# aquaskyline/SOAPdenovo-Trans

Hardware: AMD Instinct MI355X
Metric: pregraph k-mers hashed/sec (higher is better)
Workload: dtype u64

## Files before the change

### soapdenovo-trans_amd/csrc/sdt_pipeline.hip

```cpp
#include "sdt_ctx.hpp"
#include "sdt_tile.cuh"
#include "sdt_superkmer_kernels.cuh"
#include "sdt_count_plan.h"
#include "sdt_pipeline.hpp"

void sk_free(sdt_ctx *c)
{
	sdt_ctx::SkState &k = c->sk;
	void *dev[] = {k.p1.recs, k.p1.meta, k.p1.next, k.p2.recs, k.p2.meta, k.p2.next, k.cursors, k.blk, k.cnt1, k.off1, k.fill1, k.list1,
	               k.cnt2, k.off2, k.fill2, k.list2, k.kmers2, k.kpre2, k.items, k.citems, k.next_item};
	for (void *p : dev)
		if (p) (void)hipFree(p);
	void *host[] = {k.h_off1, k.h_off2, k.h_kpre2, k.h_items, k.h_citems};
	for (void *p : host)
		if (p) (void)hipHostFree(p);
	const uint64_t in_total = k.l2_in_total;
	const bool exchanged = k.exchanged;
	const uint32_t stream_flushes = k.stream_flushes;
	k = sdt_ctx::SkState();
	k.l2_in_total = in_total;
	k.exchanged = exchanged;
	k.stream_flushes = stream_flushes;
}

// ... 29 lines not shown

int sk_reset_pool1(sdt_ctx *c)
{
	sdt_ctx::SkState &k = c->sk;
	HIPCHK(hipMemsetAsync(k.p1.next, 0, 4, c->stream));
	HIPCHK(hipMemsetAsync(k.cnt1, 0, SK_NB1 * 4, c->stream));
	hipLaunchKernelGGL(k_sk_init_cursors, dim3(256), dim3(256), 0, c->stream, k.cursors, k.wgs * (uint32_t)SK_NB1, (uint32_t)SK_CAP1, k.blk, k.wgs);
	HIPCHK(hipGetLastError());
	k.pending_kmers = 0;
	return SDT_OK;
}

int sk_alloc(sdt_ctx *c, uint64_t want_kmers, uint64_t per_read)
{
	sdt_ctx::SkState &k = c->sk;
	if (want_kmers > SK_BATCH_MAX_KMERS)
		want_kmers = SK_BATCH_MAX_KMERS;
	if (k.ready && (k.cap_kmers >= want_kmers || k.cap_is_max || k.pending_kmers))
		return SDT_OK;
	if (k.ready) {
		HIPCHK(hipStreamSynchronize(c->stream));
		sk_free(c);
	}
	const int rw = sk_rec_words(c->nw), rw2 = sk_rec2_stride(c->nw);
	const int w = c->K - sk_minimizer_len(c->K) + 1;
	const double rate = 2.0 / (double)(w + 1) + 1.0 / (double)sk_max_run(c->K, c->nw);
	double run = 1.0 / rate * ((c->nw == 4 || per_read > (uint64_t)SK_SEQ_MAX_KMERS) ? 0.8 : 1.0);
	if (run > (double)per_read) run = (double)per_read;
	uint64_t div = (uint64_t)run;
	if (div < 2) div = 2;
	div = (uint64_t)clamp_int(sdt_knob_int(sdt_tuning_env("SDT_SK_POOL_DIV"), (int)div), 1, 1 << 20);
	const int mem_pct = sdt_knob_int(sdt_tuning_env("SDT_SK_POOL_MEM_PCT"), 70);
	size_t free_b = 0, total_b = 0;
	HIPCHK(sdti::mem_info(&free_b, &total_b));
	uint64_t cap = want_kmers < (1ULL << 24) ? (1ULL << 24) : want_kmers;
	k.cap_is_max = cap >= SK_BATCH_MAX_KMERS;
	const uint32_t wgs = (uint32_t)c->cu_count * 6;
	for (;; cap /= 2) {
		const uint64_t recs = cap / div;
		const uint64_t chunks1 = sdt_knob_int(sdt_test_env("SDT_SK_POOL_CHUNKS1"), 0) > 0 ? (uint64_t)sdt_knob_int(sdt_test_env("SDT_SK_POOL_CHUNKS1"), 0) : recs / SK_CAP1 + (uint64_t)wgs * SK_NB1 + 1024;
		const uint64_t items = chunks1 / SK_ITEM_CHUNKS + SK_NB1 + 1;
		const uint64_t chunks2 = chunks1 * (SK_CAP1 / SK_CAP2) + items * (SK_NB2 + SK_BLK2) + 1024;
		const uint64_t bytes = chunks1 * SK_CAP1 * rw * 8 + chunks2 * SK_CAP2 * rw2 * 8 + (chunks1 + chunks2) * 8;
		const uint64_t all = c->comm.nranks > 1 ? bytes + chunks1 * SK_CAP1 * rw * 8 * 9 / 2 : bytes;
		if (chunks2 >= (1ULL << SK_LIST2_FILL_SHIFT) - 1 || all > free_b / 100 * (uint64_t)mem_pct) {
			k.cap_is_max = true;
			if (cap <= (1ULL << 24))
				return fail(SDT_ENOMEM, "super-k-mer pools: %llu MiB needed for the smallest batch, %zu MiB free",
				            (unsigned long long)(bytes >> 20), free_b >> 20);
			continue;
		}
		k.p1.chunks = (uint32_t)chunks1;
		k.p2.chunks = (uint32_t)chunks2;
		k.items_cap = (uint32_t)items;
		break;
	}
	k.wgs = wgs;
	const double t_alloc0 = comm_now();
	HIPCHK(hipMalloc((void **)&k.p1.recs, (size_t)k.p1.chunks * SK_CAP1 * rw * 8));
	HIPCHK(hipMalloc((void **)&k.p1.meta, (size_t)k.p1.chunks * 4));
	HIPCHK(hipMalloc((void **)&k.p1.next, 64));
	HIPCHK(hipMalloc((void **)&k.p2.recs, (size_t)k.p2.chunks * SK_CAP2 * rw2 * 8));
// ... 8 lines not shown
	HIPCHK(hipMalloc((void **)&k.cnt2, SK_NBF * 4));
	HIPCHK(hipMalloc((void **)&k.off2, (SK_NBF + 1) * 4));
	HIPCHK(hipMalloc((void **)&k.fill2, SK_NBF * 4));
	HIPCHK(hipMalloc((void **)&k.list2, (size_t)k.p2.chunks * 4));
	HIPCHK(hipMalloc((void **)&k.kmers2, SK_NBF * 8));
	HIPCHK(hipMalloc((void **)&k.kpre2, (SK_NBF + 1) * 8));
	HIPCHK(hipMalloc((void **)&k.items, (size_t)k.items_cap * sizeof(SkItem)));
	HIPCHK(hipHostMalloc((void **)&k.h_off1, (SK_NB1 + 1) * 4, hipHostMallocDefault));
	HIPCHK(hipHostMalloc((void **)&k.h_off2, (SK_NBF + 1) * 4, hipHostMallocDefault));
	HIPCHK(hipHostMalloc((void **)&k.h_kpre2, (SK_NBF + 1) * 8, hipHostMallocDefault));
	HIPCHK(hipHostMalloc((void **)&k.h_items, (size_t)k.items_cap * sizeof(SkItem), hipHostMallocDefault));
	k.citems_cap = (uint32_t)SK_NBF + k.p2.chunks / SK_COUNT_ITEM_CHUNKS + 1;
	HIPCHK(hipMalloc((void **)&k.citems, (size_t)k.citems_cap * sizeof(uint4)));
	HIPCHK(hipHostMalloc((void **)&k.h_citems, (size_t)k.citems_cap * sizeof(uint4), hipHostMallocDefault));
	HIPCHK(hipMalloc((void **)&k.next_item, SK_MAX_COUNT_LAUNCHES * sizeof(uint32_t)));
	k.cap_kmers = cap;
	k.ready = true;
	if (sdt_env("SDT_TIMING"))
		fprintf(stderr, "[libsdt_gpu] super-k-mer pools for %llu k-mers per batch: %.1f GiB in %.0f ms\n", (unsigned long long)cap,
		        ((double)k.p1.chunks * SK_CAP1 * rw + (double)k.p2.chunks * SK_CAP2 * rw2) * 8 / (1 << 30), (comm_now() - t_alloc0) * 1e3);
	return sk_reset_pool1(c);
}

template <int NW, bool TRACK> static int sk_launch_count_t(sdt_ctx *c, uint32_t i0, uint32_t i1, uint32_t launch)
{
	sdt_ctx::SkState &k = c->sk;
	const size_t smem = sk_count_smem<NW, TRACK>();
	const unsigned per_cu = (unsigned)((160 * 1024) / (smem + 256));
	unsigned grid = (unsigned)c->cu_count * (per_cu < 1 ? 1 : (per_cu > 2 ? 2 : per_cu));
	if (grid > i1 - i0) grid = i1 - i0;
	HIPCHK(hipFuncSetAttribute((const void *)k_sk_count<NW, TRACK>, hipFuncAttributeMaxDynamicSharedMemorySize, (int)smem));
	hipLaunchKernelGGL((k_sk_count<NW, TRACK>), dim3(grid), dim3(SkCntGeo<NW, TRACK>::TPB), smem, c->stream, k.p2, k.list2, (const uint4 *)k.citems, i0, i1,
	                   k.next_item + launch, c->K, flat_of<NW>(c), c->d_stats);
	HIPCHK(hipGetLastError());
	return SDT_OK;
}

template <int NW> static int sk_launch_count(sdt_ctx *c, uint32_t i0, uint32_t i1, uint32_t launch)
{
	return c->d_first ? sk_launch_count_t<NW, true>(c, i0, i1, launch) : sk_launch_count_t<NW, false>(c, i0, i1, launch);
}


int sk_list1(sdt_ctx *c)
{
	sdt_ctx::SkState &k = c->sk;
	const int g = c->cu_count * 8;
	hipLaunchKernelGGL(k_sk_seal, dim3(256), dim3(256), 0, c->stream, k.cursors, k.wgs * (uint32_t)SK_NB1, k.blk, k.wgs, k.p1, (uint32_t)SK_CAP1);
	hipLaunchKernelGGL(k_sk_scan, dim3(1), dim3(1024), 0, c->stream, k.cnt1, k.off1, k.fill1, (int)SK_NB1, (const unsigned long long *)nullptr, (unsigned long long *)nullptr);
	hipLaunchKernelGGL(k_sk_chunk_place_few, dim3(g), dim3(256), 0, c->stream, k.p1, k.off1, k.fill1, k.list1, (int)SK_NB1);
	SK_CHK(hipGetLastError());
	SK_CHK(hipMemcpyAsync(k.h_off1, k.off1, (SK_NB1 + 1) * 4, hipMemcpyDeviceToHost, c->stream));
	{ const int rcw = c->comm.sync_watched(c->stream, "the chunk lists of a round"); if (rcw != SDT_OK) return rcw; }
	k.st_chunks1 = k.h_off1[SK_NB1];
	return SDT_OK;
}

int sk_split(sdt_ctx *c, const SkPool &src, const uint32_t *list, uint32_t nitems, hipEvent_t after_l2)
{
	sdt_ctx::SkState &k = c->sk;
	const int g = c->cu_count * 8;
	SK_CHK(hipMemsetAsync(k.p2.next, 0, 4, c->stream));
	SK_CHK(hipMemsetAsync(k.kmers2, 0, SK_NBF * 8, c->stream));
	SK_CHK(hipMemsetAsync(k.cnt2, 0, SK_NBF * 4, c->stream));
	if (nitems) {
		SK_CHK(hipMemcpyAsync(k.items, k.h_items, (size_t)nitems * sizeof(SkItem), hipMemcpyHostToDevice, c->stream));
		const size_t sm = c->nw == 1 ? SkL2Stage<1>::SMEM : (c->nw == 2 ? SkL2Stage<2>::SMEM : SkL2Stage<4>::SMEM);
		const void *fn = c->nw == 1 ? (const void *)k_sk_scatter_records_staged<1> : (c->nw == 2 ? (const void *)k_sk_scatter_records_staged<2> : (const void *)k_sk_scatter_records_staged<4>);
		SK_CHK(hipFuncSetAttribute(fn, hipFuncAttributeMaxDynamicSharedMemorySize, (int)sm));
		if (c->nw == 1) hipLaunchKernelGGL(k_sk_scatter_records_staged<1>, dim3(nitems), dim3(SK_L2S_TPB), sm, c->stream, src, list, k.items, k.p2, k.cnt2, k.kmers2, c->d_stats);
		else if (c->nw == 2) hipLaunchKernelGGL(k_sk_scatter_records_staged<2>, dim3(nitems), dim3(SK_L2S_TPB), sm, c->stream, src, list, k.items, k.p2, k.cnt2, k.kmers2, c->d_stats);
		else hipLaunchKernelGGL(k_sk_scatter_records_staged<4>, dim3(nitems), dim3(SK_L2S_TPB), sm, c->stream, src, list, k.items, k.p2, k.cnt2, k.kmers2, c->d_stats);
		SK_CHK(hipGetLastError());
	}
	if (after_l2)
		SK_CHK(hipEventRecord(after_l2, c->stream));
	hipLaunchKernelGGL(k_sk_scan, dim3(1), dim3(1024), 0, c->stream, k.cnt2, k.off2, k.fill2, (int)SK_NBF, (const unsigned long long *)k.kmers2, k.kpre2);
	hipLaunchKernelGGL(k_sk_chunk_place, dim3(g), dim3(256), 0, c->stream, k.p2, k.off2, k.fill2, k.list2);
	SK_CHK(hipGetLastError());
	SK_CHK(hipMemcpyAsync(k.h_kpre2, k.kpre2, (SK_NBF + 1) * 8, hipMemcpyDeviceToHost, c->stream));
	SK_CHK(hipMemcpyAsync(k.h_off2, k.off2, (SK_NBF + 1) * 4, hipMemcpyDeviceToHost, c->stream));
	return SDT_OK;
}

int sk_count_all(sdt_ctx *c)
{
	sdt_ctx::SkState &k = c->sk;
	SK_CHK(hipStreamSynchronize(c->stream));
	k.st_chunks2 = k.h_off2[SK_NBF];
	k.st_flushes++;
	k.stream_flushes++;
	k.l2_in_total += k.h_kpre2[SK_NBF];
	int rc = SDT_OK;
	uint32_t nci = 0;
	SK_CHK(hipMemsetAsync(k.next_item, 0, SK_MAX_COUNT_LAUNCHES * sizeof(uint32_t), c->stream));
// ... 101 lines not shown
		k.pending_kmers = 0;
		rc = sk_count_all(c);
	}
	if (hipEventRecord(ev2->b, c->stream) != hipSuccess && rc == SDT_OK)
		rc = fail(SDT_EHIP, "hipEventRecord failed");
	k.flushing = false;
	return rc;
}

template <int NW> static Table<NW> sk_tbl(const sdt_ctx *c, bool allow_direct)
{
	Table<NW> t = flat_of<NW>(c);
	if (!allow_direct)
		t.ent = nullptr;
	return t;
}

int sk_scatter_launch(sdt_ctx *c, const uint32_t *d_words, const uint64_t *d_offs, uint64_t nr, uint64_t max_read_len, uint64_t ob,
                             bool allow_direct)
{
	sdt_ctx::SkState &k = c->sk;
	const uint64_t per_read = max_read_len - c->K + 1;
	const SkGeo geo = sk_geo(c->K, max_read_len);
	const int m = sk_minimizer_len(c->K), ncap = sk_max_run(c->K, c->nw);
	const uint64_t ntiles = (nr + SK_TILE_READS - 1) / SK_TILE_READS;
	const unsigned grid = (unsigned)(ntiles < k.wgs ? ntiles : k.wgs);
	EventPair *ev = next_event(c);
	if (!ev)
		return fail(SDT_EHIP, "hipEventCreate failed");
	ev->kmers = nr * per_read;
	ev->stage = SDT_STAGE_SK_SCATTER;
	HIPCHK(hipEventRecord(ev->a, c->stream));
#define SK_SCATTER(NW)                                                                                                             \
	do {                                                                                                                       \
		HIPCHK(hipFuncSetAttribute((const void *)k_sk_scatter_reads<NW>, hipFuncAttributeMaxDynamicSharedMemorySize, (int)geo.smem)); \
		hipLaunchKernelGGL(k_sk_scatter_reads<NW>, dim3(grid), dim3(TPB), geo.smem, c->stream, d_words, d_offs, nr, c->K, m, ncap, \
		                   geo.mtw, geo.tile_words, geo.hv_words, geo.hv2_words, geo.bits_words, k.p1, k.cursors, k.blk, k.cnt1, sk_tbl<NW>(c, allow_direct), c->d_stats, ob, c->ord_stride); \
	} while (0)
	const int w = c->K - m + 1;
	static const bool no_seq = sdt_tuning_env("SDT_SK_STRIPS") != NULL;
	const bool seq1 = c->nw == 1 && (w & 1) && w >= 9 && w <= 21 && per_read <= (uint64_t)SK_SEQ_MAX_KMERS;
	const bool seq2 = c->nw == 2 && (w & 1) && w >= 23 && w <= 53 && per_read <= (uint64_t)SK_SEQ_MAX_KMERS;
	if ((seq1 || seq2) && !no_seq) {
		SkSeqLaunch a;
		a.words = d_words; a.offs = d_offs; a.nreads = nr; a.K = c->K; a.m = m; a.ncap = ncap;
		a.mtw = (int)(((uint64_t)SK_SEQ_TILE * max_read_len + 16 + 15) / 16) + TAIL_PAD + 1;
		a.pool = k.p1; a.cursors = k.cursors; a.blk = k.blk; a.cnt = k.cnt1; a.stats = c->d_stats;
		a.ord_base = ob; a.ord_stride = c->ord_stride; a.max_wgs = k.wgs; a.cu_count = c->cu_count; a.stream = c->stream;
		HIPCHK(seq1 ? sk_seq_launch_nw1(w, a, sk_tbl<1>(c, allow_direct)) : (w <= 33 ? sk_seq_launch_nw2_lo(w, a, sk_tbl<2>(c, allow_direct))
		            : (w <= 43 ? sk_seq_launch_nw2_mid(w, a, sk_tbl<2>(c, allow_direct)) : sk_seq_launch_nw2_hi(w, a, sk_tbl<2>(c, allow_direct)))));
	} else if (c->nw == 1) SK_SCATTER(1);
	else if (c->nw == 2) SK_SCATTER(2);
	else SK_SCATTER(4);
#undef SK_SCATTER
	HIPCHK(hipGetLastError());
	HIPCHK(hipEventRecord(ev->b, c->stream));
	k.pending_kmers += nr * per_read;
	return SDT_OK;
}
// ... 105 lines not shown
```

### soapdenovo-trans_amd/csrc/sdt_pipeline.hpp

```cpp
#pragma once
#include "sdt_ctx.hpp"

static const uint64_t SK_BATCH_MAX_KMERS = 1ULL << clamp_int(sdt_knob_int(sdt_size_env("SDT_SK_BATCH_LOG2"), 35), 24, 36);
static const uint32_t SK_ITEM_CHUNKS = (uint32_t)clamp_int(sdt_knob_int(sdt_size_env("SDT_SK_ITEM_CHUNKS"), 4096), 16, 4096);
static const uint64_t SK_COUNT_KMERS = 1ULL << clamp_int(sdt_knob_int(sdt_size_env("SDT_SK_COUNT_KMERS_LOG2"), 29), 20, 36);
static const uint32_t SK_COUNT_PACK_CHUNKS = 64;
static const uint32_t SK_COUNT_ITEM_CHUNKS = (uint32_t)clamp_int(sdt_knob_int(sdt_size_env("SDT_SK_COUNT_ITEM_CHUNKS"), 2048), 64, 1 << 24);
static const uint32_t SK_MAX_COUNT_LAUNCHES = 4096;


#define SK_CHK(expr)                                                                                   \
	do {                                                                                               \
		hipError_t e4_ = (expr);                                                                       \
		if (e4_ != hipSuccess)                                                                         \
			return fail(e4_ == hipErrorOutOfMemory ? SDT_ENOMEM : SDT_EHIP, "%s failed: %s (%s:%d)", #expr, hipGetErrorString(e4_), __FILE__, __LINE__); \
	} while (0)

struct SkGeo { int mtw, tile_words, hv_words, hv2_words, bits_words; size_t smem; };
SkGeo sk_geo(int K, uint64_t max_read_len);
bool sk_applicable(const sdt_ctx *c, uint64_t max_read_len);
int sk_reset_pool1(sdt_ctx *c);
int sk_alloc(sdt_ctx *c, uint64_t want_kmers, uint64_t per_read);
int sk_list1(sdt_ctx *c);
int sk_split(sdt_ctx *c, const SkPool &src, const uint32_t *list, uint32_t nitems, hipEvent_t after_l2);
int sk_count_all(sdt_ctx *c);
int sk_add_items(sdt_ctx::SkState &k, uint32_t &nitems, uint32_t b, uint32_t lo, uint32_t hi);
int sk_scatter_launch(sdt_ctx *c, const uint32_t *d_words, const uint64_t *d_offs, uint64_t nr, uint64_t max_read_len, uint64_t ob,
                      bool allow_direct = true);
uint64_t sk_batch_limit(const sdt_ctx *c);
int sk_scatter(sdt_ctx *c, const uint32_t *d_words, const uint64_t *d_offs, uint64_t nreads, uint64_t max_read_len);
```

### soapdenovo-trans_amd/csrc/sdt_superkmer.cuh

```cuda
#pragma once
#include "sdt_kmer.cuh"
#include "sdt_minimizer.cuh"
#include "sdt_table.cuh"

namespace sdt {

constexpr int SK_POSBITS = 22 - SK_L2BITS;
constexpr int SK_CAP1 = 32;
#ifndef SDT_SK_CAP2
#define SDT_SK_CAP2 16
#endif
constexpr int SK_CAP2 = SDT_SK_CAP2;
static_assert(SK_CAP2 == 16 || SK_CAP2 == 32, "a level-2 chunk holds 16 or 32 records");
constexpr uint32_t SK_NOCHUNK = 0xFFFFFFFFu;
constexpr int SK_MAX_RUN = 64;

template <int NW> struct SkFmt {
	static constexpr int BW = NW == 1 ? 2 : (NW == 2 ? 4 : 6);
	static constexpr int REC_WORDS = 1 + BW;
	static constexpr int CAP_BASES = 32 * BW;
#ifndef SDT_SK_REC2_PAD
#define SDT_SK_REC2_PAD 0
#endif
	static constexpr int REC2_STRIDE = (NW == 1 && SDT_SK_REC2_PAD) ? 4 : REC_WORDS;
};
constexpr uint64_t SK_MAX_READ_ORDINAL = 1ULL << 34;
constexpr int SK_MAX_READ_LEN = (1 << SK_POSBITS) - 1;

__host__ __device__ inline int sk_rec_words(int nw) { return nw == 1 ? 3 : (nw == 2 ? 5 : 7); }
__host__ __device__ inline int sk_rec2_stride(int nw) { return nw == 1 ? SkFmt<1>::REC2_STRIDE : (nw == 2 ? SkFmt<2>::REC2_STRIDE : SkFmt<4>::REC2_STRIDE); }

__host__ __device__ inline int sk_max_run(int K, int nw)
{
	const int cap = 32 * (nw == 1 ? 2 : (nw == 2 ? 4 : 6)) - K - 1;
	int n = SK_MAX_RUN;
	while (n > cap)
		n >>= 1;
	return n;
}

__host__ __device__ inline uint32_t sk_stream_mmer(const uint32_t *words, int p, int m)
{
	const int s = 2 * p, wi = s >> 5, sh = s & 31;
	const uint64_t win = ((uint64_t)words[wi] << 32) | words[wi + 1];
	return (uint32_t)((win << sh) >> (64 - 2 * m));
}

__host__ __device__ inline uint64_t sk_stream_word(const uint32_t *words, int p)
{
	const int s = 2 * p, wi = s >> 5, sh = s & 31;
	const uint64_t hi = ((uint64_t)words[wi] << 32) | words[wi + 1];
	return sh ? ((hi << sh) | ((uint64_t)words[wi + 2] >> (32 - sh))) : hi;
}

__host__ __device__ inline uint64_t sk_header(uint64_t read_ord, uint32_t pos, uint32_t l2, int n, int has_prev, int has_next)
{
	return (read_ord << 30) | ((uint64_t)(pos & (uint32_t)SK_MAX_READ_LEN) << (8 + SK_L2BITS)) | ((uint64_t)(l2 & (uint32_t)(SK_NB2 - 1)) << 8) | ((uint64_t)(n - 1) << 2) |
	       ((uint64_t)has_prev << 1) | (uint64_t)has_next;
}
__host__ __device__ inline int sk_hdr_n(uint64_t h) { return (int)((h >> 2) & 63u) + 1; }
__host__ __device__ inline int sk_hdr_prev(uint64_t h) { return (int)((h >> 1) & 1u); }
// ... 18 lines not shown
```

### soapdenovo-trans_amd/csrc/sdt_superkmer_kernels.cuh

```cuda
#pragma once

#ifndef SDT_SK_PREFETCH
#define SDT_SK_PREFETCH 1
#endif
#ifndef SDT_SK_CLAIM_BELOW
#define SDT_SK_CLAIM_BELOW 0
#endif
#ifndef SDT_SK_LOAD16
#define SDT_SK_LOAD16 1
#endif
#ifndef SDT_SK_CLAIM2_BELOW
#define SDT_SK_CLAIM2_BELOW 0
#endif
#ifndef SDT_SK_FLUSH_NUM
#define SDT_SK_FLUSH_NUM 4
#endif
#ifndef SDT_SK_NW2_TWO
#define SDT_SK_NW2_TWO 1
#endif
#ifndef SDT_SK_SEQ_FLUSH
#define SDT_SK_SEQ_FLUSH 1
#endif
#ifndef SDT_SK_CNT_TPB
#define SDT_SK_CNT_TPB 1024
// ... 356 lines not shown
#pragma unroll
		for (int t = 0; t < 16; t++)
			if (bucket[t] != 0xFFFFFFFFu)
				list[off[bucket[t]] + s_base[bucket[t]] + mine[t]] = c0 + (uint32_t)t * 256u + threadIdx.x;
		__syncthreads();
	}
}


#ifdef SDT_SK_L2_LOG
__device__ unsigned long long *g_l2_log = nullptr;
__device__ unsigned long long g_l2_log_cap = 0;
#endif

#ifndef SDT_SK_L2S_S1
#define SDT_SK_L2S_S1 4
#endif
#ifndef SDT_SK_L2S_WGS
#define SDT_SK_L2S_WGS 1
#endif
#ifndef SDT_SK_L2S_RPL
#define SDT_SK_L2S_RPL 2
#endif
template <int NW> struct SkL2Stage {
	static constexpr int S = NW == 1 ? SDT_SK_L2S_S1 : 2;
	static constexpr int GPC = SK_CAP2 / S;
	static constexpr int RPL = NW == 1 ? SDT_SK_L2S_RPL : (NW == 2 ? (SDT_SK_L2S_RPL < 2 ? SDT_SK_L2S_RPL : 2) : 1);
	static constexpr size_t SMEM = (size_t)SK_NB2 * S * SkFmt<NW>::REC_WORDS * 8;
};

template <int NW>
__global__ __launch_bounds__(SK_L2S_TPB, SDT_SK_L2S_WGS) void k_sk_scatter_records_staged(SkPool src, const uint32_t *__restrict__ list1,
                                                                         const SkItem *__restrict__ items, SkPool dst,
                                                                         uint32_t *__restrict__ g_cnt, unsigned long long *__restrict__ g_kmers, Stats *stats)
{
	constexpr int RW = SkFmt<NW>::REC_WORDS, RW2 = SkFmt<NW>::REC2_STRIDE, S = SkL2Stage<NW>::S, GPC = SkL2Stage<NW>::GPC;
	constexpr int CPT = SK_L2S_TPB / SK_CAP1;
	constexpr int D = SkL2Stage<NW>::RPL;
	extern __shared__ unsigned long long s_stage[];
	__shared__ uint32_t s_cnt[SK_NB2];
	__shared__ uint32_t s_open[SK_NB2];
	__shared__ uint32_t s_pub_open[SK_NB2], s_pub_new[SK_NB2], s_pub_g[SK_NB2];
	__shared__ unsigned char s_fill[SK_NB2], s_used[SK_NB2];
	__shared__ uint32_t s_kc[SK_NB2], s_cc[SK_NB2];
	__shared__ unsigned long long s_blk;
	const SkItem it = items[blockIdx.x];
	const int tid = threadIdx.x;
	for (int i = tid; i < SK_NB2; i += SK_L2S_TPB) {
		s_cnt[i] = 0;
		s_open[i] = SK_NOCHUNK;
		s_fill[i] = 0;
		s_used[i] = 0;
		s_kc[i] = 0;
		s_cc[i] = 0;
	}
	if (tid == 0)
		s_blk = 0;
	__syncthreads();
	uint32_t failed = 0;
	auto alloc = [&](uint32_t n) -> uint32_t {
		const uint32_t id = sk_alloc_chunks(&s_blk, dst, n, SK_BLK2);
		return id < dst.chunks && id + n <= dst.chunks ? id : SK_NOCHUNK;
	};
	auto slot_of = [&](uint32_t open, uint32_t used, uint32_t first_new, uint32_t t) -> uint64_t * {
		const uint32_t a = (open == SK_NOCHUNK ? (uint32_t)GPC : used) + t / S;
		if (a < (uint32_t)GPC)
			return dst.recs + ((size_t)open * SK_CAP2 + a * S + t % S) * RW2;
		if (first_new == SK_NOCHUNK)
			return nullptr;
		return dst.recs + ((size_t)(first_new + (a - GPC) / GPC) * SK_CAP2 + ((a - GPC) % GPC) * S + t % S) * RW2;
	};
	const uint32_t slot = (uint32_t)tid % SK_CAP1, cfirst = it.c0 + (uint32_t)tid / SK_CAP1;
	uint32_t id_a[D], id_b[D], fill_a[D];
	uint64_t rec_a[D][RW];
#pragma unroll
	for (int d = 0; d < D; d++) {
		const uint32_t ca = cfirst + (uint32_t)d * CPT, cb = ca + (uint32_t)D * CPT;
		id_a[d] = ca < it.c1 ? list1[ca] : SK_NOCHUNK;
		id_b[d] = cb < it.c1 ? list1[cb] : SK_NOCHUNK;
	}
#pragma unroll
	for (int d = 0; d < D; d++) {
		fill_a[d] = 0;
#pragma unroll
		for (int i = 0; i < RW; i++)
			rec_a[d][i] = 0;
		if (id_a[d] != SK_NOCHUNK) {
			fill_a[d] = src.meta[id_a[d]] >> 24;
			sk_load_record<RW>(src.recs + ((size_t)id_a[d] * SK_CAP1 + slot) * RW, rec_a[d]);
		}
	}
	const uint32_t nsweep = (it.c1 - it.c0 + CPT - 1) / CPT;
	for (uint32_t sw = 0; sw < nsweep; sw += (uint32_t)D) {
		uint64_t rec[D][RW];
		uint32_t b2[D], t[D];
		bool valid[D];
#pragma unroll
		for (int d = 0; d < D; d++) {
			const uint32_t ci = cfirst + (sw + (uint32_t)d) * CPT;
#pragma unroll
			for (int i = 0; i < RW; i++)
				rec[d][i] = rec_a[d][i];
			const uint32_t fill = ci < it.c1 ? fill_a[d] : 0u;
			id_a[d] = id_b[d];
			const uint32_t cn = ci + 2u * (uint32_t)D * CPT;
			id_b[d] = cn < it.c1 ? list1[cn] : SK_NOCHUNK;
			if (id_a[d] != SK_NOCHUNK) {
				fill_a[d] = src.meta[id_a[d]] >> 24;
				sk_load_record<RW>(src.recs + ((size_t)id_a[d] * SK_CAP1 + slot) * RW, rec_a[d]);
			}
			valid[d] = slot < fill;
			b2[d] = 0;
			t[d] = 0;
			if (valid[d]) {
				b2[d] = sk_hdr_l2(rec[d][0]);
				t[d] = atomicAdd(&s_cnt[b2[d]], 1u);
				atomicAdd(&s_kc[b2[d]], (uint32_t)sk_hdr_n(rec[d][0]));
			}
		}
		__syncthreads();
		for (int i = tid; i < SK_NB2; i += SK_L2S_TPB) {
			const uint32_t f = s_fill[i], total = s_cnt[i];
			if (total == f)
				continue;
			const uint32_t G = total / S, left = total - G * S;
			const uint32_t open = s_open[i], used = open == SK_NOCHUNK ? (uint32_t)GPC : s_used[i];
			const uint32_t room = (uint32_t)GPC - used;
			uint32_t first_new = SK_NOCHUNK;
			if (G > room) {
				const uint32_t nnew = (G - room + GPC - 1) / GPC;
				first_new = alloc(nnew);
				if (first_new != SK_NOCHUNK) {
					for (uint32_t j = 0; j < nnew; j++)
						dst.meta[first_new + j] = (it.b1 * SK_NB2 + (uint32_t)i) | ((uint32_t)SK_CAP2 << 24);
					s_cc[i] += nnew;
				}
			}
			s_pub_open[i] = open;
			s_pub_new[i] = first_new;
			s_pub_g[i] = used | (G << 8);
			if (G && f) {
				for (uint32_t j = 0; j < f; j++) {
					uint64_t old[RW];
#pragma unroll
					for (int w = 0; w < RW; w++)
						old[w] = s_stage[((size_t)i * S + j) * RW + w];
					uint64_t *p = slot_of(open, used, first_new, j);
					if (p) sk_store_record2<NW>(p, old);
					else failed++;
				}
			}
			if (G) {
				const uint32_t a_end = used + G;
				if (a_end <= (uint32_t)GPC) {
					s_used[i] = (unsigned char)a_end;
				} else if (first_new != SK_NOCHUNK) {
					s_open[i] = first_new + (a_end - GPC - 1) / GPC;
					s_used[i] = (unsigned char)((a_end - GPC - 1) % GPC + 1);
				} else {
					s_open[i] = SK_NOCHUNK;
					s_used[i] = 0;
				}
			}
			s_fill[i] = (unsigned char)left;
			s_cnt[i] = left;
		}
		__syncthreads();
#pragma unroll
		for (int d = 0; d < D; d++) {
			if (!valid[d])
				continue;
			const uint32_t g = s_pub_g[b2[d]], G = g >> 8, used = g & 0xFFu;
			if (t[d] / S < G) {
				uint64_t *p = slot_of(s_pub_open[b2[d]], used, s_pub_new[b2[d]], t[d]);
				if (p) sk_store_record2<NW>(p, rec[d]);
				else failed++;
			} else {
				const uint32_t at = t[d] - G * S;
#pragma unroll
				for (int i = 0; i < RW; i++)
					s_stage[((size_t)b2[d] * S + at) * RW + i] = rec[d][i];
			}
		}
	}
	__syncthreads();
	for (int i = tid; i < SK_NB2; i += SK_L2S_TPB) {
		const uint32_t f = s_fill[i];
		uint32_t open = s_open[i], used = open == SK_NOCHUNK ? (uint32_t)GPC : s_used[i];
		if (f) {
			if (used == (uint32_t)GPC) {
				open = alloc(1);
				used = 0;
				if (open != SK_NOCHUNK)
					s_cc[i]++;
			}
			if (open != SK_NOCHUNK) {
				for (uint32_t j = 0; j < f; j++) {
					uint64_t rec[RW];
#pragma unroll
					for (int w = 0; w < RW; w++)
						rec[w] = s_stage[((size_t)i * S + j) * RW + w];
					sk_store_record2<NW>(dst.recs + ((size_t)open * SK_CAP2 + used * S + j) * RW2, rec);
				}
			} else {
				failed += f;
			}
		}
		if (open != SK_NOCHUNK)
			dst.meta[open] = (it.b1 * SK_NB2 + (uint32_t)i) | ((used * S + f) << 24);
		if (s_kc[i])
			atomicAdd(&g_kmers[it.b1 * SK_NB2 + i], (unsigned long long)s_kc[i]);
		if (s_cc[i])
			atomicAdd(&g_cnt[it.b1 * SK_NB2 + i], s_cc[i]);
	}
	__syncthreads();
	{
		const unsigned long long blk = s_blk;
		const uint32_t next = (uint32_t)blk, end = (uint32_t)(blk >> 32);
		for (uint32_t id = next + (uint32_t)tid; id < end && id < dst.chunks; id += SK_L2S_TPB)
			dst.meta[id] = SK_DEAD;
	}
	if (failed)
		atomicAdd(&stats->probe_fail, (unsigned long long)failed);
}

// ... 103 lines not shown
	uint64_t v = 0;
	uint32_t cnt = f[2] & 0xFFFFu;
#pragma unroll
	for (int b = 0; b < 4; b++) {
		const uint32_t l = (f[b >> 1] >> ((b & 1) * 16)) & 0xFFFFu, r = (f[4 - (b >> 1)] >> (16 - (b & 1) * 16)) & 0xFFFFu;
		cnt += l;
		v |= (uint64_t)(l > 63u ? 63u : l) << (6 * b);
		v |= (uint64_t)(r > 63u ? 63u : r) << (24 + 6 * b);
	}
	return v | ((uint64_t)cnt << 48);
}

__device__ inline uint64_t sk_weighted_val(uint32_t w, uint32_t prev, uint32_t next)
{
	const uint64_t c = w > 63u ? 63u : w;
	uint64_t v = (uint64_t)(w & 0xFFFFu) << 48;
	if (prev < 4u) v |= c << (6 * prev);
	if (next < 4u) v |= c << (24 + 6 * next);
	return v;
}

constexpr uint32_t SK_CNT_MAX_SINCE = 65535;

template <int NW, bool TRACK>
__global__ __launch_bounds__((SkCntGeo<NW, TRACK>::TPB), (SkCntGeo<NW, TRACK>::WAVES_PER_SIMD)) void k_sk_count(SkPool pool, const uint32_t *__restrict__ list2, const uint4 *__restrict__ items,
                                                         uint32_t item0, uint32_t item1, uint32_t *__restrict__ next_item, int K,
                                                         Table<NW> tbl, Stats *stats)
{
	using G = SkCntGeo<NW, TRACK>;
	constexpr int BW = SkFmt<NW>::BW, RW = SkFmt<NW>::REC_WORDS, SLOTS = G::SLOTS;
	constexpr uint32_t FLUSH_AT = G::FLUSH_AT, MAXFILL = G::MAXFILL;
	constexpr int SK_CNT_TPB = G::TPB;
	constexpr int TR = G::TILE;
	constexpr int CPT = TR / SK_CAP2;
	constexpr int NWAVES = TR / 64;
	constexpr uint32_t REP = G::REP, REP_EMPTY = 0xFFFFFFFFu;
	extern __shared__ unsigned long long sm64[];
	unsigned long long *s_h0 = sm64;
	uint32_t *s_w = (uint32_t *)(s_h0 + TR);
	uint32_t *s_pre = s_w + TR;
	unsigned short *s_map = (unsigned short *)(s_pre + TR + 2);
	unsigned short *s_idx = s_map + TR;
	uint32_t *s_rep = s_pre;
	uint32_t *s_words = (uint32_t *)((char *)s_pre + G::REGION);
	unsigned long long *s_key = (unsigned long long *)(s_words + LDS_LEAD + TR * BW * 2 + TAIL_PAD);
	unsigned long long *s_ord = s_key + NW * SLOTS;
	uint32_t *s_f = (uint32_t *)(s_ord + (TRACK ? SLOTS : 0));
// ... 49 lines not shown
		}
		if ((tid & 63) == 0) {
			if (claimed) atomicAdd(&s_stat[ST_CLAIMED], claimed);
			if (failed) atomicAdd(&s_stat[ST_FAILED], failed);
			if (merges) atomicAdd(&s_stat[ST_MERGES], merges);
		}
		stores_pending = true;
	};
	for (;;) {
		if (tid == 0) {
			s_item = item0 + atomicAdd(next_item, 1u);
			s_spilled = 0;
		}
		__syncthreads();
		const uint32_t item = (uint32_t)__builtin_amdgcn_readfirstlane((int)s_item);
		__syncthreads();
		if (item >= item1)
			break;
		const uint4 it = items[item];
		const uint32_t ity = (uint32_t)__builtin_amdgcn_readfirstlane((int)it.y);
		const uint32_t c0 = (uint32_t)__builtin_amdgcn_readfirstlane((int)it.x), c1 = ity & 0x7FFFFFFFu;
		const bool whole = (ity >> 31) != 0;
		auto rec_ptr = [&](uint32_t e, uint32_t t) -> const uint64_t * {
			return pool.recs + ((size_t)(e & ((1u << SK_LIST2_FILL_SHIFT) - 1u)) * SK_CAP2 + t % SK_CAP2) * SkFmt<NW>::REC2_STRIDE;
		};
		auto rec_ok = [&](uint32_t e, uint32_t t) -> bool { return e != SK_NOCHUNK && t % SK_CAP2 <= (e >> SK_LIST2_FILL_SHIFT); };
		auto ent_row = [&](uint32_t t) -> uint32_t * { return s_ent + (t % 3u) * CPT; };
		if (tid < CPT) {
			ent_row(0)[tid] = c0 + (uint32_t)tid < c1 ? list2[c0 + tid] : SK_NOCHUNK;
			ent_row(1)[tid] = c0 + CPT + (uint32_t)tid < c1 ? list2[c0 + CPT + tid] : SK_NOCHUNK;
		}
		__syncthreads();
		uint32_t tile_no = 0;
		uint32_t since = 0;
		SK_TICK(0);
		for (uint32_t cb = c0; cb < c1; cb += CPT) {
			uint32_t ot_ = (uint32_t)tid;
			asm volatile("" : "+v"(ot_));
			const int ot = (int)ot_;
			uint32_t n = 0;
			uint64_t h0 = 0;
			uint64_t nx[RW];
			uint32_t ring_e = SK_NOCHUNK, pf = 0;
			const uint32_t e = ot < TR ? ent_row(tile_no)[ot / SK_CAP2] : SK_NOCHUNK;
			const uint32_t e1 = ot < TR ? ent_row(tile_no + 1)[ot / SK_CAP2] : SK_NOCHUNK;
			const bool ok = rec_ok(e, ot);
			sk_load_record<RW>(ok ? rec_ptr(e, ot) : pool.recs, nx);
			const bool ring_ok = ot < CPT && cb + 2 * CPT + (uint32_t)ot < c1;
			ring_e = (list2 + cb)[ring_ok ? 2 * CPT + ot : 0];
			if (!ring_ok)
				ring_e = SK_NOCHUNK;
			if (SDT_SK_PREFETCH)
				pf = *(const uint32_t *)(rec_ok(e1, ot) ? rec_ptr(e1, ot) : pool.recs);
			if (ot < TR) {
				if (ok) {
					h0 = nx[0];
					n = (uint32_t)sk_hdr_n(h0);
#pragma unroll
					for (int i = 0; i < BW; i++) {
						words[ot * BW * 2 + 2 * i] = (uint32_t)(nx[1 + i] >> 32);
						words[ot * BW * 2 + 2 * i + 1] = (uint32_t)nx[1 + i];
					}
				}
				s_h0[ot] = h0;
				s_w[ot] = 1;
			}
			for (uint32_t i = ot; i < REP; i += SK_CNT_TPB)
				s_rep[i] = REP_EMPTY;
			__syncthreads();
			bool distinct = false;
			if (n) {
				distinct = true;
				uint32_t x = (uint32_t)h0 & SK_HDR_KIND_MASK;
#pragma unroll
				for (int i = 0; i < BW; i++) {
					x = __builtin_rotateleft32(x, 5) ^ (uint32_t)nx[1 + i];
// ... 291 lines not shown
```

Before: 94.28 billion.

## Pack level-2 super-k-mer records into two words for single-word keys

Adds a compact 2-word level-2 record format for 1-word keys without first-occurrence tracking. The header's low byte is folded into the unused low bits of the second base word, and the maximum super-k-mer run is capped so the bases fit in 60 bases. The change cuts record bytes written by the scatter kernel and read by the count kernel, and so reduces memory traffic and pool size. In exchange, shorter runs produce more records, so pool sizing is scaled up. The scatter loop is also restructured to prefetch with clamped indices instead of branches.

```diff
diff --git a/soapdenovo-trans_amd/csrc/sdt_pipeline.hip b/soapdenovo-trans_amd/csrc/sdt_pipeline.hip
--- a/soapdenovo-trans_amd/csrc/sdt_pipeline.hip
+++ b/soapdenovo-trans_amd/csrc/sdt_pipeline.hip
@@ -75,9 +75,13 @@
 		HIPCHK(hipStreamSynchronize(c->stream));
 		sk_free(c);
 	}
-	const int rw = sk_rec_words(c->nw), rw2 = sk_rec2_stride(c->nw);
+	const bool compact = sk_compact(c);
+	const int rw = sk_rec_words(c->nw), rw2 = sk_rec2_stride(c->nw, compact);
 	const int w = c->K - sk_minimizer_len(c->K) + 1;
+	const bool strips = c->nw == 4 || per_read > (uint64_t)SK_SEQ_MAX_KMERS;
+	const int cap_c = strips ? sk_pow2_floor(sk_max_run(c->K, c->nw, compact)) : sk_max_run(c->K, c->nw, compact);
 	const double rate = 2.0 / (double)(w + 1) + 1.0 / (double)sk_max_run(c->K, c->nw);
+	const double more = compact ? (2.0 / (double)(w + 1) + 1.0 / (double)cap_c) / rate : 1.0;
 	double run = 1.0 / rate * ((c->nw == 4 || per_read > (uint64_t)SK_SEQ_MAX_KMERS) ? 0.8 : 1.0);
 	if (run > (double)per_read) run = (double)per_read;
 	uint64_t div = (uint64_t)run;
@@ -90,7 +94,7 @@
 	k.cap_is_max = cap >= SK_BATCH_MAX_KMERS;
 	const uint32_t wgs = (uint32_t)c->cu_count * 6;
 	for (;; cap /= 2) {
-		const uint64_t recs = cap / div;
+		const uint64_t recs = (uint64_t)((double)(cap / div) * more);
 		const uint64_t chunks1 = sdt_knob_int(sdt_test_env("SDT_SK_POOL_CHUNKS1"), 0) > 0 ? (uint64_t)sdt_knob_int(sdt_test_env("SDT_SK_POOL_CHUNKS1"), 0) : recs / SK_CAP1 + (uint64_t)wgs * SK_NB1 + 1024;
 		const uint64_t items = chunks1 / SK_ITEM_CHUNKS + SK_NB1 + 1;
 		const uint64_t chunks2 = chunks1 * (SK_CAP1 / SK_CAP2) + items * (SK_NB2 + SK_BLK2) + 1024;
@@ -145,15 +149,15 @@
 	return sk_reset_pool1(c);
 }
 
-template <int NW, bool TRACK> static int sk_launch_count_t(sdt_ctx *c, uint32_t i0, uint32_t i1, uint32_t launch)
+template <int NW, bool TRACK, bool COMPACT> static int sk_launch_count_t(sdt_ctx *c, uint32_t i0, uint32_t i1, uint32_t launch)
 {
 	sdt_ctx::SkState &k = c->sk;
 	const size_t smem = sk_count_smem<NW, TRACK>();
 	const unsigned per_cu = (unsigned)((160 * 1024) / (smem + 256));
 	unsigned grid = (unsigned)c->cu_count * (per_cu < 1 ? 1 : (per_cu > 2 ? 2 : per_cu));
 	if (grid > i1 - i0) grid = i1 - i0;
-	HIPCHK(hipFuncSetAttribute((const void *)k_sk_count<NW, TRACK>, hipFuncAttributeMaxDynamicSharedMemorySize, (int)smem));
-	hipLaunchKernelGGL((k_sk_count<NW, TRACK>), dim3(grid), dim3(SkCntGeo<NW, TRACK>::TPB), smem, c->stream, k.p2, k.list2, (const uint4 *)k.citems, i0, i1,
+	HIPCHK(hipFuncSetAttribute((const void *)k_sk_count<NW, TRACK, COMPACT>, hipFuncAttributeMaxDynamicSharedMemorySize, (int)smem));
+	hipLaunchKernelGGL((k_sk_count<NW, TRACK, COMPACT>), dim3(grid), dim3(SkCntGeo<NW, TRACK>::TPB), smem, c->stream, k.p2, k.list2, (const uint4 *)k.citems, i0, i1,
 	                   k.next_item + launch, c->K, flat_of<NW>(c), c->d_stats);
 	HIPCHK(hipGetLastError());
 	return SDT_OK;
@@ -161,7 +165,12 @@
 
 template <int NW> static int sk_launch_count(sdt_ctx *c, uint32_t i0, uint32_t i1, uint32_t launch)
 {
-	return c->d_first ? sk_launch_count_t<NW, true>(c, i0, i1, launch) : sk_launch_count_t<NW, false>(c, i0, i1, launch);
+	if (c->d_first)
+		return sk_launch_count_t<NW, true, false>(c, i0, i1, launch);
+	if constexpr (NW == 1)
+		if (sk_compact(c))
+			return sk_launch_count_t<1, false, true>(c, i0, i1, launch);
+	return sk_launch_count_t<NW, false, false>(c, i0, i1, launch);
 }
 
 
@@ -188,12 +197,17 @@
 	SK_CHK(hipMemsetAsync(k.cnt2, 0, SK_NBF * 4, c->stream));
 	if (nitems) {
 		SK_CHK(hipMemcpyAsync(k.items, k.h_items, (size_t)nitems * sizeof(SkItem), hipMemcpyHostToDevice, c->stream));
-		const size_t sm = c->nw == 1 ? SkL2Stage<1>::SMEM : (c->nw == 2 ? SkL2Stage<2>::SMEM : SkL2Stage<4>::SMEM);
-		const void *fn = c->nw == 1 ? (const void *)k_sk_scatter_records_staged<1> : (c->nw == 2 ? (const void *)k_sk_scatter_records_staged<2> : (const void *)k_sk_scatter_records_staged<4>);
-		SK_CHK(hipFuncSetAttribute(fn, hipFuncAttributeMaxDynamicSharedMemorySize, (int)sm));
-		if (c->nw == 1) hipLaunchKernelGGL(k_sk_scatter_records_staged<1>, dim3(nitems), dim3(SK_L2S_TPB), sm, c->stream, src, list, k.items, k.p2, k.cnt2, k.kmers2, c->d_stats);
-		else if (c->nw == 2) hipLaunchKernelGGL(k_sk_scatter_records_staged<2>, dim3(nitems), dim3(SK_L2S_TPB), sm, c->stream, src, list, k.items, k.p2, k.cnt2, k.kmers2, c->d_stats);
-		else hipLaunchKernelGGL(k_sk_scatter_records_staged<4>, dim3(nitems), dim3(SK_L2S_TPB), sm, c->stream, src, list, k.items, k.p2, k.cnt2, k.kmers2, c->d_stats);
+#define SK_L2_LAUNCH(NW, COMPACT)                                                                                                   \
+		do {                                                                                                                        \
+			const size_t sm = SkL2Stage<NW, COMPACT>::SMEM;                                                                         \
+			SK_CHK(hipFuncSetAttribute((const void *)k_sk_scatter_records_staged<NW, COMPACT>, hipFuncAttributeMaxDynamicSharedMemorySize, (int)sm)); \
+			hipLaunchKernelGGL((k_sk_scatter_records_staged<NW, COMPACT>), dim3(nitems), dim3(SK_L2S_TPB), sm, c->stream, src, list, k.items, k.p2, k.cnt2, k.kmers2, c->d_stats); \
+		} while (0)
+		if (c->nw == 1 && sk_compact(c)) SK_L2_LAUNCH(1, true);
+		else if (c->nw == 1) SK_L2_LAUNCH(1, false);
+		else if (c->nw == 2) SK_L2_LAUNCH(2, false);
+		else SK_L2_LAUNCH(4, false);
+#undef SK_L2_LAUNCH
 		SK_CHK(hipGetLastError());
 	}
 	if (after_l2)
@@ -341,7 +355,7 @@
 	sdt_ctx::SkState &k = c->sk;
 	const uint64_t per_read = max_read_len - c->K + 1;
 	const SkGeo geo = sk_geo(c->K, max_read_len);
-	const int m = sk_minimizer_len(c->K), ncap = sk_max_run(c->K, c->nw);
+	const int m = sk_minimizer_len(c->K), ncap = sk_max_run(c->K, c->nw, sk_compact(c));
 	const uint64_t ntiles = (nr + SK_TILE_READS - 1) / SK_TILE_READS;
 	const unsigned grid = (unsigned)(ntiles < k.wgs ? ntiles : k.wgs);
 	EventPair *ev = next_event(c);
@@ -353,7 +367,7 @@
 #define SK_SCATTER(NW)                                                                                                             \
 	do {                                                                                                                       \
 		HIPCHK(hipFuncSetAttribute((const void *)k_sk_scatter_reads<NW>, hipFuncAttributeMaxDynamicSharedMemorySize, (int)geo.smem)); \
-		hipLaunchKernelGGL(k_sk_scatter_reads<NW>, dim3(grid), dim3(TPB), geo.smem, c->stream, d_words, d_offs, nr, c->K, m, ncap, \
+		hipLaunchKernelGGL(k_sk_scatter_reads<NW>, dim3(grid), dim3(TPB), geo.smem, c->stream, d_words, d_offs, nr, c->K, m, sk_pow2_floor(ncap), \
 		                   geo.mtw, geo.tile_words, geo.hv_words, geo.hv2_words, geo.bits_words, k.p1, k.cursors, k.blk, k.cnt1, sk_tbl<NW>(c, allow_direct), c->d_stats, ob, c->ord_stride); \
 	} while (0)
 	const int w = c->K - m + 1;
diff --git a/soapdenovo-trans_amd/csrc/sdt_pipeline.hpp b/soapdenovo-trans_amd/csrc/sdt_pipeline.hpp
--- a/soapdenovo-trans_amd/csrc/sdt_pipeline.hpp
+++ b/soapdenovo-trans_amd/csrc/sdt_pipeline.hpp
@@ -16,6 +16,8 @@
 			return fail(e4_ == hipErrorOutOfMemory ? SDT_ENOMEM : SDT_EHIP, "%s failed: %s (%s:%d)", #expr, hipGetErrorString(e4_), __FILE__, __LINE__); \
 	} while (0)
 
+static inline bool sk_compact(const sdt_ctx *c) { return sdt::sk_compact2(c->nw, (c->flags & SDT_FLAG_TRACK_FIRST) != 0); }
+
 struct SkGeo { int mtw, tile_words, hv_words, hv2_words, bits_words; size_t smem; };
 SkGeo sk_geo(int K, uint64_t max_read_len);
 bool sk_applicable(const sdt_ctx *c, uint64_t max_read_len);
diff --git a/soapdenovo-trans_amd/csrc/sdt_sk_record2.h b/soapdenovo-trans_amd/csrc/sdt_sk_record2.h
--- /dev/null
+++ b/soapdenovo-trans_amd/csrc/sdt_sk_record2.h
@@ -0,0 +1,56 @@
+#pragma once
+#include <stdint.h>
+
+#if defined(__HIPCC__)
+#define SDT_SK_HD __host__ __device__
+#else
+#define SDT_SK_HD
+#endif
+
+namespace sdt {
+
+constexpr int SK_MAX_RUN = 64;
+constexpr int SK_REC2C_WORDS = 2;
+constexpr int SK_REC2C_BASES = 60;
+constexpr int SK_REC2C_MAX_RUN = 32;
+
+#ifndef SDT_SK_COMPACT2
+#define SDT_SK_COMPACT2 1
+#endif
+SDT_SK_HD inline bool sk_compact2(int nw, bool track_first) { return SDT_SK_COMPACT2 && nw == 1 && !track_first; }
+
+SDT_SK_HD inline int sk_max_run(int K, int nw, bool compact = false)
+{
+	const int cap = 32 * (nw == 1 ? 2 : (nw == 2 ? 4 : 6)) - K - 1;
+	int n = SK_MAX_RUN;
+	while (n > cap)
+		n >>= 1;
+	if (compact && nw == 1) {
+		const int c = SK_REC2C_BASES - K - 1;
+		const int m = c < SK_REC2C_MAX_RUN ? c : SK_REC2C_MAX_RUN;
+		if (m < n)
+			n = m;
+	}
+	return n;
+}
+SDT_SK_HD inline int sk_pow2_floor(int n)
+{
+	int p = 1;
+	while (2 * p <= n)
+		p *= 2;
+	return p;
+}
+
+SDT_SK_HD inline void sk_pack2(uint64_t hdr, uint64_t b0, uint64_t b1, uint64_t &w0, uint64_t &w1)
+{
+	w0 = b0;
+	w1 = (b1 & ~0xFFULL) | (hdr & 0xFFULL);
+}
+SDT_SK_HD inline void sk_unpack2(uint64_t w0, uint64_t w1, uint64_t &hdr, uint64_t &b0, uint64_t &b1)
+{
+	hdr = w1 & 0xFFULL;
+	b0 = w0;
+	b1 = w1 & ~0xFFULL;
+}
+
+}
diff --git a/soapdenovo-trans_amd/csrc/sdt_superkmer.cuh b/soapdenovo-trans_amd/csrc/sdt_superkmer.cuh
--- a/soapdenovo-trans_amd/csrc/sdt_superkmer.cuh
+++ b/soapdenovo-trans_amd/csrc/sdt_superkmer.cuh
@@ -2,6 +2,7 @@
 #include "sdt_kmer.cuh"
 #include "sdt_minimizer.cuh"
 #include "sdt_table.cuh"
+#include "sdt_sk_record2.h"
 
 namespace sdt {
 
@@ -13,7 +14,6 @@
 constexpr int SK_CAP2 = SDT_SK_CAP2;
 static_assert(SK_CAP2 == 16 || SK_CAP2 == 32, "a level-2 chunk holds 16 or 32 records");
 constexpr uint32_t SK_NOCHUNK = 0xFFFFFFFFu;
-constexpr int SK_MAX_RUN = 64;
 
 template <int NW> struct SkFmt {
 	static constexpr int BW = NW == 1 ? 2 : (NW == 2 ? 4 : 6);
@@ -28,15 +28,9 @@
 constexpr int SK_MAX_READ_LEN = (1 << SK_POSBITS) - 1;
 
 __host__ __device__ inline int sk_rec_words(int nw) { return nw == 1 ? 3 : (nw == 2 ? 5 : 7); }
-__host__ __device__ inline int sk_rec2_stride(int nw) { return nw == 1 ? SkFmt<1>::REC2_STRIDE : (nw == 2 ? SkFmt<2>::REC2_STRIDE : SkFmt<4>::REC2_STRIDE); }
-
-__host__ __device__ inline int sk_max_run(int K, int nw)
+__host__ __device__ inline int sk_rec2_stride(int nw, bool compact)
 {
-	const int cap = 32 * (nw == 1 ? 2 : (nw == 2 ? 4 : 6)) - K - 1;
-	int n = SK_MAX_RUN;
-	while (n > cap)
-		n >>= 1;
-	return n;
+	return compact ? SK_REC2C_WORDS : (nw == 1 ? SkFmt<1>::REC2_STRIDE : (nw == 2 ? SkFmt<2>::REC2_STRIDE : SkFmt<4>::REC2_STRIDE));
 }
 
 __host__ __device__ inline uint32_t sk_stream_mmer(const uint32_t *words, int p, int m)
diff --git a/soapdenovo-trans_amd/csrc/sdt_superkmer_kernels.cuh b/soapdenovo-trans_amd/csrc/sdt_superkmer_kernels.cuh
--- a/soapdenovo-trans_amd/csrc/sdt_superkmer_kernels.cuh
+++ b/soapdenovo-trans_amd/csrc/sdt_superkmer_kernels.cuh
@@ -402,22 +402,34 @@
 #ifndef SDT_SK_L2S_RPL
 #define SDT_SK_L2S_RPL 2
 #endif
-template <int NW> struct SkL2Stage {
+template <int NW, bool COMPACT = false> struct SkL2Stage {
+	static_assert(!COMPACT || NW == 1, "the compact level-2 record is the 1-word keys'");
 	static constexpr int S = NW == 1 ? SDT_SK_L2S_S1 : 2;
 	static constexpr int GPC = SK_CAP2 / S;
 	static constexpr int RPL = NW == 1 ? SDT_SK_L2S_RPL : (NW == 2 ? (SDT_SK_L2S_RPL < 2 ? SDT_SK_L2S_RPL : 2) : 1);
-	static constexpr size_t SMEM = (size_t)SK_NB2 * S * SkFmt<NW>::REC_WORDS * 8;
+	static constexpr int RWS = COMPACT ? SK_REC2C_WORDS : SkFmt<NW>::REC_WORDS;
+	static constexpr int RW2 = COMPACT ? SK_REC2C_WORDS : SkFmt<NW>::REC2_STRIDE;
+	static constexpr size_t SMEM = (size_t)SK_NB2 * S * RWS * 8;
 };
 
-template <int NW>
+template <int NW, bool COMPACT> __device__ inline void sk_store_staged(uint64_t *dst, const uint64_t (&rec)[SkL2Stage<NW, COMPACT>::RWS])
+{
+	if constexpr (COMPACT)
+		*reinterpret_cast<ulonglong2 *>(dst) = make_ulonglong2(rec[0], rec[1]);
+	else
+		sk_store_record2<NW>(dst, rec);
+}
+
+template <int NW, bool COMPACT>
 __global__ __launch_bounds__(SK_L2S_TPB, SDT_SK_L2S_WGS) void k_sk_scatter_records_staged(SkPool src, const uint32_t *__restrict__ list1,
                                                                          const SkItem *__restrict__ items, SkPool dst,
                                                                          uint32_t *__restrict__ g_cnt, unsigned long long *__restrict__ g_kmers, Stats *stats)
 {
-	constexpr int RW = SkFmt<NW>::REC_WORDS, RW2 = SkFmt<NW>::REC2_STRIDE, S = SkL2Stage<NW>::S, GPC = SkL2Stage<NW>::GPC;
+	using L2 = SkL2Stage<NW, COMPACT>;
+	constexpr int RW = SkFmt<NW>::REC_WORDS, RWS = L2::RWS, RW2 = L2::RW2, S = L2::S, GPC = L2::GPC;
 	constexpr int CPT = SK_L2S_TPB / SK_CAP1;
-	constexpr int D = SkL2Stage<NW>::RPL;
-	extern __shared__ unsigned long long s_stage[];
+	constexpr int D = L2::RPL;
+	extern __shared__ __attribute__((aligned(16))) unsigned long long s_stage[];
 	__shared__ uint32_t s_cnt[SK_NB2];
 	__shared__ uint32_t s_open[SK_NB2];
 	__shared__ uint32_t s_pub_open[SK_NB2], s_pub_new[SK_NB2], s_pub_g[SK_NB2];
@@ -451,51 +463,69 @@
 		return dst.recs + ((size_t)(first_new + (a - GPC) / GPC) * SK_CAP2 + ((a - GPC) % GPC) * S + t % S) * RW2;
 	};
 	const uint32_t slot = (uint32_t)tid % SK_CAP1, cfirst = it.c0 + (uint32_t)tid / SK_CAP1;
-	uint32_t id_a[D], id_b[D], fill_a[D];
+	uint32_t id_b[D], meta_a[D];
 	uint64_t rec_a[D][RW];
-#pragma unroll
-	for (int d = 0; d < D; d++) {
-		const uint32_t ca = cfirst + (uint32_t)d * CPT, cb = ca + (uint32_t)D * CPT;
-		id_a[d] = ca < it.c1 ? list1[ca] : SK_NOCHUNK;
-		id_b[d] = cb < it.c1 ? list1[cb] : SK_NOCHUNK;
-	}
-#pragma unroll
-	for (int d = 0; d < D; d++) {
-		fill_a[d] = 0;
-#pragma unroll
-		for (int i = 0; i < RW; i++)
-			rec_a[d][i] = 0;
-		if (id_a[d] != SK_NOCHUNK) {
-			fill_a[d] = src.meta[id_a[d]] >> 24;
-			sk_load_record<RW>(src.recs + ((size_t)id_a[d] * SK_CAP1 + slot) * RW, rec_a[d]);
+	{
+		uint32_t id_a[D];
+#pragma unroll
+		for (int d = 0; d < D; d++) {
+			const uint32_t ca = cfirst + (uint32_t)d * CPT, cb = ca + (uint32_t)D * CPT;
+			id_a[d] = list1[ca < it.c1 ? ca : it.c0];
+			id_b[d] = list1[cb < it.c1 ? cb : it.c0];
+		}
+#pragma unroll
+		for (int d = 0; d < D; d++) {
+			const uint32_t ca = cfirst + (uint32_t)d * CPT;
+			const uint32_t id = ca < it.c1 ? id_a[d] : 0u;
+			meta_a[d] = src.meta[id];
+			sk_load_record<RW>(src.recs + ((size_t)id * SK_CAP1 + slot) * RW, rec_a[d]);
 		}
 	}
 	const uint32_t nsweep = (it.c1 - it.c0 + CPT - 1) / CPT;
 	for (uint32_t sw = 0; sw < nsweep; sw += (uint32_t)D) {
-		uint64_t rec[D][RW];
+		uint64_t rec[D][RWS];
 		uint32_t b2[D], t[D];
 		bool valid[D];
 #pragma unroll
 		for (int d = 0; d < D; d++) {
+			asm volatile("" : "+v"(id_b[d]), "+v"(meta_a[d]));
+#pragma unroll
+			for (int i = 0; i < RW; i++)
+				asm volatile("" : "+v"(rec_a[d][i]));
+		}
+		uint64_t hdr[D];
+		uint32_t fill[D];
+#pragma unroll
+		for (int d = 0; d < D; d++) {
 			const uint32_t ci = cfirst + (sw + (uint32_t)d) * CPT;
-#pragma unroll
-			for (int i = 0; i < RW; i++)
-				rec[d][i] = rec_a[d][i];
-			const uint32_t fill = ci < it.c1 ? fill_a[d] : 0u;
-			id_a[d] = id_b[d];
-			const uint32_t cn = ci + 2u * (uint32_t)D * CPT;
-			id_b[d] = cn < it.c1 ? list1[cn] : SK_NOCHUNK;
-			if (id_a[d] != SK_NOCHUNK) {
-				fill_a[d] = src.meta[id_a[d]] >> 24;
-				sk_load_record<RW>(src.recs + ((size_t)id_a[d] * SK_CAP1 + slot) * RW, rec_a[d]);
-			}
-			valid[d] = slot < fill;
+			hdr[d] = rec_a[d][0];
+			fill[d] = ci < it.c1 ? meta_a[d] >> 24 : 0u;
+			if constexpr (COMPACT) {
+				sk_pack2(rec_a[d][0], rec_a[d][1], rec_a[d][2], rec[d][0], rec[d][1]);
+			} else {
+#pragma unroll
+				for (int i = 0; i < RW; i++)
+					rec[d][i] = rec_a[d][i];
+			}
+		}
+#pragma unroll
+		for (int d = 0; d < D; d++) {
+			const uint32_t ci = cfirst + (sw + (uint32_t)d) * CPT;
+			const uint32_t c1n = ci + (uint32_t)D * CPT, c2n = ci + 2u * (uint32_t)D * CPT;
+			const uint32_t id = c1n < it.c1 ? id_b[d] : 0u;
+			id_b[d] = list1[c2n < it.c1 ? c2n : it.c0];
+			meta_a[d] = src.meta[id];
+			sk_load_record<RW>(src.recs + ((size_t)id * SK_CAP1 + slot) * RW, rec_a[d]);
+		}
+#pragma unroll
+		for (int d = 0; d < D; d++) {
+			valid[d] = slot < fill[d];
 			b2[d] = 0;
 			t[d] = 0;
 			if (valid[d]) {
-				b2[d] = sk_hdr_l2(rec[d][0]);
+				b2[d] = sk_hdr_l2(hdr[d]);
 				t[d] = atomicAdd(&s_cnt[b2[d]], 1u);
-				atomicAdd(&s_kc[b2[d]], (uint32_t)sk_hdr_n(rec[d][0]));
+				atomicAdd(&s_kc[b2[d]], (uint32_t)sk_hdr_n(hdr[d]));
 			}
 		}
 		__syncthreads();
@@ -521,12 +551,12 @@
 			s_pub_g[i] = used | (G << 8);
 			if (G && f) {
 				for (uint32_t j = 0; j < f; j++) {
-					uint64_t old[RW];
-#pragma unroll
-					for (int w = 0; w < RW; w++)
-						old[w] = s_stage[((size_t)i * S + j) * RW + w];
+					uint64_t old[RWS];
+#pragma unroll
+					for (int w = 0; w < RWS; w++)
+						old[w] = s_stage[((size_t)i * S + j) * RWS + w];
 					uint64_t *p = slot_of(open, used, first_new, j);
-					if (p) sk_store_record2<NW>(p, old);
+					if (p) sk_store_staged<NW, COMPACT>(p, old);
 					else failed++;
 				}
 			}
@@ -553,13 +583,13 @@
 			const uint32_t g = s_pub_g[b2[d]], G = g >> 8, used = g & 0xFFu;
 			if (t[d] / S < G) {
 				uint64_t *p = slot_of(s_pub_open[b2[d]], used, s_pub_new[b2[d]], t[d]);
-				if (p) sk_store_record2<NW>(p, rec[d]);
+				if (p) sk_store_staged<NW, COMPACT>(p, rec[d]);
 				else failed++;
 			} else {
 				const uint32_t at = t[d] - G * S;
 #pragma unroll
-				for (int i = 0; i < RW; i++)
-					s_stage[((size_t)b2[d] * S + at) * RW + i] = rec[d][i];
+				for (int i = 0; i < RWS; i++)
+					s_stage[((size_t)b2[d] * S + at) * RWS + i] = rec[d][i];
 			}
 		}
 	}
@@ -576,11 +606,11 @@
 			}
 			if (open != SK_NOCHUNK) {
 				for (uint32_t j = 0; j < f; j++) {
-					uint64_t rec[RW];
-#pragma unroll
-					for (int w = 0; w < RW; w++)
-						rec[w] = s_stage[((size_t)i * S + j) * RW + w];
-					sk_store_record2<NW>(dst.recs + ((size_t)open * SK_CAP2 + used * S + j) * RW2, rec);
+					uint64_t rec[RWS];
+#pragma unroll
+					for (int w = 0; w < RWS; w++)
+						rec[w] = s_stage[((size_t)i * S + j) * RWS + w];
+					sk_store_staged<NW, COMPACT>(dst.recs + ((size_t)open * SK_CAP2 + used * S + j) * RW2, rec);
 				}
 			} else {
 				failed += f;
@@ -730,7 +760,7 @@
 
 constexpr uint32_t SK_CNT_MAX_SINCE = 65535;
 
-template <int NW, bool TRACK>
+template <int NW, bool TRACK, bool COMPACT>
 __global__ __launch_bounds__((SkCntGeo<NW, TRACK>::TPB), (SkCntGeo<NW, TRACK>::WAVES_PER_SIMD)) void k_sk_count(SkPool pool, const uint32_t *__restrict__ list2, const uint4 *__restrict__ items,
                                                          uint32_t item0, uint32_t item1, uint32_t *__restrict__ next_item, int K,
                                                          Table<NW> tbl, Stats *stats)
@@ -826,7 +856,7 @@
 		const uint32_t c0 = (uint32_t)__builtin_amdgcn_readfirstlane((int)it.x), c1 = ity & 0x7FFFFFFFu;
 		const bool whole = (ity >> 31) != 0;
 		auto rec_ptr = [&](uint32_t e, uint32_t t) -> const uint64_t * {
-			return pool.recs + ((size_t)(e & ((1u << SK_LIST2_FILL_SHIFT) - 1u)) * SK_CAP2 + t % SK_CAP2) * SkFmt<NW>::REC2_STRIDE;
+			return pool.recs + ((size_t)(e & ((1u << SK_LIST2_FILL_SHIFT) - 1u)) * SK_CAP2 + t % SK_CAP2) * (COMPACT ? SK_REC2C_WORDS : SkFmt<NW>::REC2_STRIDE);
 		};
 		auto rec_ok = [&](uint32_t e, uint32_t t) -> bool { return e != SK_NOCHUNK && t % SK_CAP2 <= (e >> SK_LIST2_FILL_SHIFT); };
 		auto ent_row = [&](uint32_t t) -> uint32_t * { return s_ent + (t % 3u) * CPT; };
@@ -849,13 +879,21 @@
 			const uint32_t e = ot < TR ? ent_row(tile_no)[ot / SK_CAP2] : SK_NOCHUNK;
 			const uint32_t e1 = ot < TR ? ent_row(tile_no + 1)[ot / SK_CAP2] : SK_NOCHUNK;
 			const bool ok = rec_ok(e, ot);
-			sk_load_record<RW>(ok ? rec_ptr(e, ot) : pool.recs, nx);
+			ulonglong2 cx = make_ulonglong2(0ULL, 0ULL);
+			if constexpr (COMPACT) {
+				static_assert(!COMPACT || (NW == 1 && !TRACK), "compact records carry no ordinals");
+				cx = *reinterpret_cast<const ulonglong2 *>(ok ? rec_ptr(e, ot) : pool.recs);
+			} else {
+				sk_load_record<RW>(ok ? rec_ptr(e, ot) : pool.recs, nx);
+			}
 			const bool ring_ok = ot < CPT && cb + 2 * CPT + (uint32_t)ot < c1;
 			ring_e = (list2 + cb)[ring_ok ? 2 * CPT + ot : 0];
 			if (!ring_ok)
 				ring_e = SK_NOCHUNK;
 			if (SDT_SK_PREFETCH)
 				pf = *(const uint32_t *)(rec_ok(e1, ot) ? rec_ptr(e1, ot) : pool.recs);
+			if constexpr (COMPACT)
+				sk_unpack2(cx.x, cx.y, nx[0], nx[1], nx[RW - 1]);
 			if (ot < TR) {
 				if (ok) {
 					h0 = nx[0];
```

Measured after the change: 99.28 billion, median of 6. 1.05x the previous value.
